# vsislab/Controllable_XGating

Hardware: AMD Instinct MI355X
Metric: decoder timesteps/sec (train fwd+bwd) at batch 128, MSRVTT 26x1536+1024 (higher is better)
Workload: dtype f32; 1 GPU; configs[1]: 1xMI355X batch 128 per GPU teacher-forced XE train, 26 frames x (1536+1024), hidden 512, att 1536, emb 468, vocab 20000, seq_len 20 (T=21), fp32; global_batch=128, per_gpu_batch=128, parallelism=dp1, gemm_precision=fp32, zero_grad=fused into the update, launch=eager kernel launches

## Files before the change

controllable_xgating_amd/csrc/xg_heads.hip:

```cpp
#include "xg_common.h"
#include "xg_kernels.h"
#include "xg_select.h"
#include <type_traits>
#include <cstdlib>

namespace {

constexpr int RT = 1024;

__device__ __forceinline__ float block_max(float v, float* red) {
    v = wave_max(v);
    const int lane = threadIdx.x & 63, wave = threadIdx.x >> 6;
    __syncthreads();
    if (lane == 0) red[wave] = v;
    __syncthreads();
    float r = red[0];
    for (int i = 1; i < (int)(blockDim.x >> 6); ++i) r = fmaxf(r, red[i]);
    return r;
}
__device__ __forceinline__ float block_sum(float v, float* red) {
    v = wave_sum(v);
    const int lane = threadIdx.x & 63, wave = threadIdx.x >> 6;
    __syncthreads();
    if (lane == 0) red[wave] = v;
// ... 147 lines not shown
    s = (mx == -INFINITY) ? 0.f : s * expf(mx - gmx);
    s = block_sum(s, red);
    if (threadIdx.x == 0) {
        const float lse = gmx + logf(s);
        lse_out[i] = lse;
        const float m = mask[(size_t)b * T + t] * (mask2 ? mask2[(size_t)b * T + t] : 1.f);
        const int64_t tg = tgt_of(seq, b, t, T, roll);
        atomicAdd(sums2, -(x[tg] - lse) * m);
        atomicAdd(sums2 + 1, m);
    }
}
__global__ void __launch_bounds__(RT) xent_fwd_kernel(const float* __restrict__ logits, int ld, const int64_t* seq,
                                                        const float* mask, const float* mask2, int B, int T, int V,
                                                        int roll, float* lse_out, float* sums2, int row0) {
    __shared__ float red[RT / 64];
    const int i = row0 + blockIdx.x, t = i / B, b = i % B;
    const float* x = logits + (size_t)i * ld;
    float mx = -INFINITY, s = 0.f;
    for (int v0 = threadIdx.x; v0 < V; v0 += 8 * RT) {
        float xv[8];
#pragma unroll
        for (int j = 0; j < 8; ++j) { const int v = v0 + j * RT; xv[j] = v < V ? x[v] : -INFINITY; }
        float bm = xv[0];
#pragma unroll
        for (int j = 1; j < 8; ++j) bm = fmaxf(bm, xv[j]);
        if (bm > mx) { s *= expf(mx - bm); mx = bm; }
        if (mx > -INFINITY) {
#pragma unroll
            for (int j = 0; j < 8; ++j) s += expf(xv[j] - mx);
        }
    }
    xent_row_finish(mx, s, red, x, i, b, t, T, seq, mask, mask2, roll, lse_out, sums2);
}
template <int NV4>
__global__ void __launch_bounds__(RT) xent_fwd_reg_kernel(const float* __restrict__ logits, int ld, const int64_t* seq,
                                                            const float* mask, const float* mask2, int B, int T, int V,
                                                            int roll, float* lse_out, float* sums2, int row0) {
    __shared__ float red[RT / 64];
    const int i = row0 + blockIdx.x, t = i / B, b = i % B;
    const float* x = logits + (size_t)i * ld;
    float4 xv[NV4];
#pragma unroll
    for (int j = 0; j < NV4; ++j) {
        const int v = (threadIdx.x + j * RT) * 4;
        if (v + 3 < V) xv[j] = *reinterpret_cast<const float4*>(x + v);
        else {
            xv[j].x = v < V ? x[v] : -INFINITY;         xv[j].y = v + 1 < V ? x[v + 1] : -INFINITY;
            xv[j].z = v + 2 < V ? x[v + 2] : -INFINITY; xv[j].w = -INFINITY;
        }
    }
    float mx = -INFINITY;
#pragma unroll
    for (int j = 0; j < NV4; ++j) mx = fmaxf(fmaxf(mx, fmaxf(xv[j].x, xv[j].y)), fmaxf(xv[j].z, xv[j].w));
    float s = 0.f;
    if (mx > -INFINITY) {
#pragma unroll
        for (int j = 0; j < NV4; ++j) s += (expf(xv[j].x - mx) + expf(xv[j].y - mx)) + (expf(xv[j].z - mx) + expf(xv[j].w - mx));
    }
    xent_row_finish(mx, s, red, x, i, b, t, T, seq, mask, mask2, roll, lse_out, sums2);
}
template <bool BF>
__global__ void __launch_bounds__(RT) xent_bwd_kernel(float* __restrict__ logits, int ld, const int64_t* seq,
                                                        const float* mask, const float* mask2, int B, int T, int V,
                                                        int roll, const float* lse, const float* sums2,
                                                        const float* scale_dev, float scale, int row0, unsigned short* d16) {
    const int i = row0 + blockIdx.x, t = i / B, b = i % B;
    float* x = logits + (size_t)i * ld;
    const float m = mask[(size_t)b * T + t] * (mask2 ? mask2[(size_t)b * T + t] : 1.f);
    const float coef = (scale_dev ? scale_dev[0] : 1.f) * scale * m / sums2[1];
    const int64_t tg = tgt_of(seq, b, t, T, roll);
    const float l = lse[i];
    for (int v = threadIdx.x; v < V; v += RT) {
        const float pv = expf(x[v] - l);
        const float gv = coef * (pv - (v == tg ? 1.f : 0.f));
        x[v] = gv;
        if (BF) {
            unsigned u = __float_as_uint(gv);
            u += 0x7FFFu + ((u >> 16) & 1u);
            d16[(size_t)i * ld + v] = (unsigned short)(u >> 16);
        }
    }
}

template <int NV4, bool BF>
__global__ void __launch_bounds__(RT) xent_bwd_reg_kernel(float* __restrict__ logits, int ld, const int64_t* seq,
                                                            const float* mask, const float* mask2, int B, int T, int V,
                                                            int roll, const float* lse, const float* sums2,
                                                            const float* scale_dev, float scale, int row0, unsigned short* d16) {
    const int i = row0 + blockIdx.x, t = i / B, b = i % B;
    float* x = logits + (size_t)i * ld;
    float4 xv[NV4];
#pragma unroll
// ... 1037 lines not shown
    else if (npt <= 16) hipLaunchKernelGGL((log_softmax_reg_kernel<16>), dim3(rows), dim3(RT), 0, st, in, ldin, out, ldout, V, inner, outer, pm);
    else if (npt <= 24) hipLaunchKernelGGL((log_softmax_reg_kernel<24>), dim3(rows), dim3(RT), 0, st, in, ldin, out, ldout, V, inner, outer, pm);
    else hipLaunchKernelGGL(log_softmax_kernel, dim3(rows), dim3(RT), 0, st, in, ldin, out, ldout, V, inner, outer, pm);
    XG_CHECK_LAUNCH();
    return XG_OK;
}
int xgk_log_softmax_bwd(hipStream_t st, const float* dlogp, const float* logp, int ldp, float* dlogits, int ldd,
                        int rows, int V, int inner, int outer, int permute) {
    if (rows <= 0) return XG_OK;
    const int npt = xg_cdiv(V, RT);
    if (npt <= 8) hipLaunchKernelGGL((log_softmax_bwd_reg_kernel<8>), dim3(rows), dim3(RT), 0, st, dlogp, logp, ldp, dlogits, ldd, V, inner, outer, permute);
    else if (npt <= 16) hipLaunchKernelGGL((log_softmax_bwd_reg_kernel<16>), dim3(rows), dim3(RT), 0, st, dlogp, logp, ldp, dlogits, ldd, V, inner, outer, permute);
    else if (npt <= 24) hipLaunchKernelGGL((log_softmax_bwd_reg_kernel<24>), dim3(rows), dim3(RT), 0, st, dlogp, logp, ldp, dlogits, ldd, V, inner, outer, permute);
    else hipLaunchKernelGGL(log_softmax_bwd_kernel, dim3(rows), dim3(RT), 0, st, dlogp, logp, ldp, dlogits, ldd, V, inner, outer, permute);
    XG_CHECK_LAUNCH();
    return XG_OK;
}
int xgk_nll_fwd(hipStream_t st, const float* logp, const int64_t* target, const float* mask, const float* mask2,
                int B, int T, int V, int roll, float* out2) {
    if (hipMemsetAsync(out2, 0, 2 * sizeof(float), st) != hipSuccess) return XG_EHIP;
    hipLaunchKernelGGL(nll_fwd_kernel, dim3(xg_cdiv(B * T, 256)), dim3(256), 0, st, logp, target, mask, mask2, B, T, V,
                       roll, out2);
    XG_CHECK_LAUNCH();
    return XG_OK;
}
int xgk_nll_bwd(hipStream_t st, const int64_t* target, const float* mask, const float* mask2, int B, int T, int V,
                int roll, const float* sums, float scale, const float* scale_dev, float* dlogp) {
    if (hipMemsetAsync(dlogp, 0, sizeof(float) * (size_t)B * T * V, st) != hipSuccess) return XG_EHIP;
    hipLaunchKernelGGL(nll_bwd_kernel, dim3(xg_cdiv(B * T, 256)), dim3(256), 0, st, target, mask, mask2, B, T, V, roll,
                       sums, scale, scale_dev, dlogp);
    XG_CHECK_LAUNCH();
    return XG_OK;
}
int xgk_xent_fwd(hipStream_t st, const float* logits, int ld, const int64_t* seq, const float* mask,
                 const float* mask2, int B, int T, int V, int roll, float* lse, float* sums2, int row0, int nrows,
                 bool zero_sums) {
    if (zero_sums && hipMemsetAsync(sums2, 0, 2 * sizeof(float), st) != hipSuccess) return XG_EHIP;
    if (nrows < 0) nrows = B * T - row0;
    if (nrows <= 0) return XG_OK;
    const bool al = ((uintptr_t)logits % 16 == 0) && ld % 4 == 0;
#define XG_XENT_REG(NV4_) hipLaunchKernelGGL((xent_fwd_reg_kernel<NV4_>), dim3(nrows), dim3(RT), 0, st, logits, ld, seq, mask, mask2, B, T, V, roll, lse, sums2, row0)
    if (al && V <= 2 * 4096) XG_XENT_REG(2);
    else if (al && V <= 5 * 4096) XG_XENT_REG(5);
    else if (al && V <= 8 * 4096) XG_XENT_REG(8);
    else hipLaunchKernelGGL(xent_fwd_kernel, dim3(nrows), dim3(RT), 0, st, logits, ld, seq, mask, mask2, B, T, V, roll, lse, sums2, row0);
#undef XG_XENT_REG
    XG_CHECK_LAUNCH();
    return XG_OK;
}
int xgk_xent_bwd(hipStream_t st, float* logits_inout, int ld, const int64_t* seq, const float* mask,
                 const float* mask2, int B, int T, int V, int roll, const float* lse, const float* sums2,
                 const float* scale_dev, float scale, int row0, int nrows, unsigned short* d16) {
    if (nrows < 0) nrows = B * T - row0;
    if (nrows <= 0) return XG_OK;
    const bool al = ((uintptr_t)logits_inout % 16 == 0) && ld % 4 == 0 && (!d16 || (uintptr_t)d16 % 8 == 0);
#define XG_XENT_BREG(NV4_) do { \
        if (d16) hipLaunchKernelGGL((xent_bwd_reg_kernel<NV4_, true>), dim3(nrows), dim3(RT), 0, st, logits_inout, ld, seq, mask, mask2, B, T, V, \
                                    roll, lse, sums2, scale_dev, scale, row0, d16); \
        else hipLaunchKernelGGL((xent_bwd_reg_kernel<NV4_, false>), dim3(nrows), dim3(RT), 0, st, logits_inout, ld, seq, mask, mask2, B, T, V, \
                                roll, lse, sums2, scale_dev, scale, row0, d16); } while (0)
    if (al && V > 1024 && V <= 2 * 4096) XG_XENT_BREG(2);
    else if (al && V > 1024 && V <= 5 * 4096) XG_XENT_BREG(5);
    else if (al && V > 1024 && V <= 8 * 4096) XG_XENT_BREG(8);
    else if (d16) hipLaunchKernelGGL(xent_bwd_kernel<true>, dim3(nrows), dim3(RT), 0, st, logits_inout, ld, seq, mask, mask2, B, T, V, roll,
                                     lse, sums2, scale_dev, scale, row0, d16);
    else hipLaunchKernelGGL(xent_bwd_kernel<false>, dim3(nrows), dim3(RT), 0, st, logits_inout, ld, seq, mask, mask2, B, T, V, roll,
                            lse, sums2, scale_dev, scale, row0, d16);
#undef XG_XENT_BREG
    XG_CHECK_LAUNCH();
    return XG_OK;
}
int xgk_choose(hipStream_t st, const float* logp, int B, int V, int mode, const float* uniforms,
               const int64_t* forced, int64_t forced_stride, float temperature, int64_t* tok, float* tok_logp) {
    hipLaunchKernelGGL(choose_kernel, dim3(B), dim3(RT), 0, st, logp, V, mode, uniforms, forced, forced_stride,
// ... 124 lines not shown
```

controllable_xgating_amd/csrc/xg_kernels.h:

```cpp
#pragma once
#include "xg_common.h"
#include "xg_select.h"
#include "xg_beam_core.h"
#include "xg_gemm_route.h"
#include <cstddef>
#include <type_traits>

int xgk_gemm(hipStream_t st, int mode, bool transA, bool transB, int M, int N, int K, const float* A, int lda,
             const float* B, int ldb, float* C, int ldc, const float* bias, bool relu, bool accumulate);
int xgk_gemm_cs(hipStream_t st, int mode, bool transA, bool transB, int M, int N, int K, const float* A, int lda,
                const float* B, int ldb, float* C, int ldc, const float* bias, bool relu, bool accumulate, float* cs1, float* cs2,
                float* cs3);
int xgk_gemm_x(hipStream_t st, int mode, bool transA, bool transB, int M, int N, int K, const float* A, const unsigned short* A16,
               int lda, const float* B, const unsigned short* B16, int ldb, float* C, int ldc, const float* bias, bool relu,
               bool accumulate, float* cs1 = nullptr, float* cs2 = nullptr, float* cs3 = nullptr);
struct XgGemmPtrs {
    const float* A; const float* B; float* C; const float* bias;
    const unsigned short* A16; const unsigned short* B16;
    float* cs[3];
};
#ifdef XG_DIAG
int xgk_gemm_run(hipStream_t st, bool wide_forced, int mode, bool transA, bool transB, int M, int N, int K, int lda, int ldb, int ldc,
                 bool relu, bool accumulate, const XgGemmPtrs& p, const XgGemmTuning* tune = nullptr, XgGemmRoute* launched = nullptr);
#else
// ... 196 lines not shown
int xgk_attn_fwd(hipStream_t st, const float* p, const float* vproj, const float* V, const float* w, float* alpha,
                 float* af, int B, int K, int R, int A, bool half_cu = false);
int xgk_attn_fwd_group(hipStream_t st, const float* p, const float* vproj, const float* V, const float* w, float* alpha,
                       float* af, int B, int S, int K, int R, int A);
int xgk_attn_bwd(hipStream_t st, const float* daf, int lddaf, const float* p, const float* vproj, const float* V,
                 const float* w, const float* alpha, float* de, float* dp, int B, int K, int R, int A);
int xgk_attn_bwd_post(hipStream_t st, const float* P , const float* vproj, const float* w,
                      const float* DE , float* dvproj, float* dw, int T, int B, int K, int A);
int xgk_attn_post_dV(hipStream_t st, const float* P, const float* vproj, const float* w, const float* DE, float* dvproj, float* dw,
                     const float* ALPHA, const float* DAF, int lddaf, int64_t daf_tstride, float* dV, int T, int B, int K, int A, int R);
int xgk_attn_dV(hipStream_t st, const float* ALPHA , const float* DAF , int lddaf,
                int64_t daf_tstride, float* dV, int T, int B, int K, int R, bool accumulate);
constexpr int XGK_ATTN_BWD_GROUP = 4;
int xgk_attn_bwd_group(hipStream_t st, const float* daf, int lddaf, const float* p, const float* vproj, const float* V, const float* w,
                       const float* alpha, float* de, float* dp, int B, int Q, int K, int R, int A);
int xgk_attn_bwd_group_form(const float* daf, int lddaf, const float* p, const float* vproj, const float* V, const float* w,
                            const float* dp, int K, int R, int A);
int xgk_attn_post_dV_group(hipStream_t st, const float* P , const float* vproj, const float* w, const float* DE ,
                           float* dvproj, float* dw, const float* ALPHA , const float* DAF, int lddaf, int64_t daf_tstride,
                           float* dV, int T, int B, int Q, int K, int A, int R);
int xgk_rows_sum_group(hipStream_t st, const float* in, float* out, int B, int Q, int R);

int xgk_log_softmax(hipStream_t st, const float* in, int ldin, float* out, int ldout, int rows, int V, int inner,
                    int outer, bool permute);
int xgk_log_softmax_bwd(hipStream_t st, const float* dlogp, const float* logp, int ldp, float* dlogits, int ldd,
                        int rows, int V, int inner, int outer, int permute);
int xgk_nll_fwd(hipStream_t st, const float* logp, const int64_t* target, const float* mask, const float* mask2,
                int B, int T, int V, int roll, float* out2);
int xgk_nll_bwd(hipStream_t st, const int64_t* target, const float* mask, const float* mask2, int B, int T, int V,
                int roll, const float* sums, float scale, const float* scale_dev, float* dlogp);
int xgk_xent_fwd(hipStream_t st, const float* logits, int ld, const int64_t* seq, const float* mask,
                 const float* mask2, int B, int T, int V, int roll, float* lse, float* sums2, int row0 = 0,
                 int nrows = -1, bool zero_sums = true);
int xgk_xent_bwd(hipStream_t st, float* logits_inout, int ld, const int64_t* seq, const float* mask,
                 const float* mask2, int B, int T, int V, int roll, const float* lse, const float* sums2,
                 const float* scale_dev, float scale, int row0 = 0, int nrows = -1, unsigned short* d16 = nullptr);
int xgk_choose(hipStream_t st, const float* logp, int B, int V, int mode, const float* uniforms,
               const int64_t* forced, int64_t forced_stride, float temperature, int64_t* tok, float* tok_logp);
int xgk_rollout_step(hipStream_t st, int B, const RollStepArgs& a);
int xgk_rollout_finalize(hipStream_t st, const int32_t* maxf, int32_t* n_steps, int Tm1, int nparts);
bool xgk_vocab_select_ok(int B, int R, int V, const float* H, int ldh, const float* W);
int xgk_vocab_tile_width(int V);
int xgk_vocab_part(hipStream_t st, int B, int R, int V, const float* H, int ldh, const float* W, const float* bias, float* logits,
                   int wr_rows, float* part, float temperature);
RollSelectArgs xgk_roll_select_args(const RollStepArgs& r, const float* part);
int xgk_roll_select(hipStream_t st, int B, const RollStepArgs& r, const float* part);
int xgk_rollout_trunc(hipStream_t st, int B, const RollStepArgs& r, const RollTruncArgs& q);
int xgk_rollout_dlogits_lse(hipStream_t st, float* logits, const float* lse, const int64_t* tok, const float* dslp,
                            int64_t dstride, int B, int V, int steps);
constexpr int XG_COMPACT_MAX = 48;
struct CompactEntry { float* dst; const float* src; int64_t dst_block, src_pitch, total; };
struct CompactArgs { int n; int start[XG_COMPACT_MAX + 1]; CompactEntry e[XG_COMPACT_MAX]; };
int xgk_compact(hipStream_t st, CompactArgs& a);
int xgk_ss_select(hipStream_t st, const int64_t* seq, int T, int t, int B, const float* u_sel, float ss_prob,
                  const int64_t* sampled, int64_t* tok);
struct SsChoiceArgs {
    const float* logits;
    const float* part;
    const float* u_sel;
    const float* u_tok;
    const int64_t* seq;
    const float* table;
    int64_t* tok;
    int64_t* tok_out;
    float* xt;
    float ss_prob;
// ... 39 lines not shown
```

controllable_xgating_amd/csrc/xg_model.hip:

```cpp
#include "xg_common.h"
#include <cstring>
#include "xg_kernels.h"
#include "../../include/xgate_beam.h"
#include "../../include/xgate_control.h"
#include "../../include/xgate_truncate.h"
#include "../../include/xgate_score.h"
#include "../../include/xgate_beam_control.h"
#include "../../include/xgate_beam_allow.h"
#include "../../include/xgate_beam_rules.h"
#include "../../include/xgate_beam_diverse.h"
#include "../../include/xgate_pair.h"
#include "../../include/xgate_train_video.h"
#include "../../include/xgate_scst_video.h"
#include "../../include/xgate_ss.h"

#include <new>
#include <cstdlib>

namespace {

constexpr int XG_NEV = 64, XG_NRING = 56;
struct XgAux { uint32_t magic; int device; hipStream_t s = nullptr, s2 = nullptr; hipEvent_t ev[XG_NEV]; };
constexpr uint32_t XG_AUX_MAGIC = 0x58474158u;
XgAux* aux_of(const XgRun* run) {
// ... 149 lines not shown
    do { if (hipMemsetAsync((ptr), 0, sizeof(float) * (size_t)(nfloats), (st)) != hipSuccess) return XG_EHIP; } while (0)
#define COPY(st, dst, src, nfloats) \
    do { if (hipMemcpyAsync((dst), (src), sizeof(float) * (size_t)(nfloats), hipMemcpyDeviceToDevice, (st)) != hipSuccess) return XG_EHIP; } while (0)
inline int record_prof(void* event, hipStream_t st) {
    return (!event || hipEventRecord(static_cast<hipEvent_t>(event), st) == hipSuccess) ? XG_OK : XG_EHIP;
}

inline int gemm_nn(hipStream_t st, int mode, int M, int N, int Kc, const float* dY, int lddy, const float* W, int ldw,
                   float* dX, int lddx, bool acc) {
    return xgk_gemm(st, mode, false, false, M, N, Kc, dY, lddy, W, ldw, dX, lddx, nullptr, false, acc);
}
inline int gemm_tn(hipStream_t st, int mode, int Mrows, int N, int K, const float* dY, int lddy, const float* X, int ldx,
                   float* dW, int lddw) {
    return xgk_gemm(st, mode, true, false, N, K, Mrows, dY, lddy, X, ldx, dW, lddw, nullptr, false, true);
}

inline int gemm_tn_cs(hipStream_t st, int mode, int Mrows, int N, int K, const float* dY, int lddy, const float* X, int ldx,
                      float* dW, int lddw, float* b1, float* b2 = nullptr, float* b3 = nullptr) {
    return xgk_gemm_cs(st, mode, true, false, N, K, Mrows, dY, lddy, X, ldx, dW, lddw, nullptr, false, true, b1, b2, b3);
}

inline const unsigned short* m16(const Ws& w, const float* p) {
    return (w.gm == 1 && w.sh16 && p >= w.base_f && p < w.end_f) ? w.sh16 + (p - w.base_f) : nullptr;
}
inline int cvt16(hipStream_t st, const Ws& w, const float* p, size_t n) {
    if (w.gm != 1 || n == 0) return XG_OK;
    if (!w.sh16) return XG_OK;
    const unsigned short* dst = m16(w, p);
    if (!dst) return XG_EINVAL;
    return xgk_cvt_bf16(st, p, const_cast<unsigned short*>(dst), n);
}
inline const unsigned short* w16(const Ws& w, int which) {
    return (w.gm == 1 && w.packed && w.pk.dtype == 1) ? w.pk.w16[which] : nullptr;
}
inline int lin16(hipStream_t st, int mode, int M, int N, int K, const float* X, const unsigned short* X16, int ldx, const float* W,
                 const unsigned short* W16, const float* bias, float* Y, int ldy, bool relu = false, bool acc = false) {
    return xgk_gemm_x(st, mode, false, true, M, N, K, X, X16, ldx, W, W16, K, Y, ldy, bias, relu, acc);
}
inline int nn16(hipStream_t st, int mode, int M, int N, int Kc, const float* dY, const unsigned short* dY16, int lddy, const float* W,
                const unsigned short* W16, int ldw, float* dX, int lddx, bool acc) {
    return xgk_gemm_x(st, mode, false, false, M, N, Kc, dY, dY16, lddy, W, W16, ldw, dX, lddx, nullptr, false, acc);
}
inline int tn16(hipStream_t st, int mode, int Mrows, int N, int K, const float* dY, const unsigned short* dY16, int lddy, const float* X,
                const unsigned short* X16, int ldx, float* dW, int lddw, float* b1 = nullptr, float* b2 = nullptr, float* b3 = nullptr) {
    return xgk_gemm_x(st, mode, true, false, N, K, Mrows, dY, dY16, lddy, X, X16, ldx, dW, lddw, nullptr, false, true, b1, b2, b3);
}

inline SkSeg seg_nt(const float* A, int lda, const float* W, int ldw, int K) {
    SkSeg s{}; s.A = A; s.B = W; s.lda = lda; s.ldb = ldw; s.K = K; s.b_ncontig = 0; return s;
}
inline SkSeg seg_nn(const float* dY, int lddy, const float* W, int ldw, int Kc) {
    SkSeg s{}; s.A = dY; s.B = W; s.lda = lddy; s.ldb = ldw; s.K = Kc; s.b_ncontig = 1; return s;
}
inline SkSeg seg_nt(const Ws& w, int which, const float* A, int lda, const float* W, int ldw, int K) {
    SkSeg s = seg_nt(A, lda, W, ldw, K);
    if (w.packed) { s.Bp = w.pk.m[which]; s.nck = w.pk.nck[which]; }
    return s;
}
inline SkSeg seg_nn(const Ws& w, int which, const float* dY, int lddy, const float* W, int ldw, int Kc) {
    SkSeg s = seg_nn(dY, lddy, W, ldw, Kc);
    if (w.packed) { s.Bp = w.pk.m[which]; s.nck = w.pk.nck[which]; }
    return s;
}
inline void allow_split(SkArgs& sk, int j, const Ws& w) { sk.job[j].ksplit_ok = 1; sk.job[j].tickets = w.tickets + j * SKPART_INTS; }
inline int zero_tickets(hipStream_t st, const Ws& w, int njobs) {
    return hipMemsetAsync(w.tickets, 0, sizeof(int32_t) * njobs * SKPART_INTS, st) == hipSuccess ? XG_OK : XG_EHIP;
// ... 520 lines not shown
    const size_t BR = (size_t)B * R;
    if (!step_scratch_ok(w, false, rows_per_video > 0) || (rows_per_video > 0) != (enc != nullptr)) return XG_EINVAL;
    const Ws& vw = enc ? *enc : w;
    if (!enc) XG_TRY(init_and_vproj(ss, d, p, x.feat_mask, w));
    XG_TRY(zero_dsync(st, w));
    XG_TRY(ss.join());
    const int th = (ss.overlap() && T >= 4) ? T / 2 : 0;
    const bool fwd_bg = th > 0 && w.gm == 0;
    static const char* chunk_env = xg_diag_env("XG_LOGIT_CHUNK");
    int chunk = 3, tail = 2;
    if (chunk_env) sscanf(chunk_env, "%d,%d", &chunk, &tail);
    const bool chunked = fwd_bg && chunk > 0 && tail > 0;
    const int last_cut = chunked ? T - tail : th;
    int done = 0;
    *logit_rows_done = 0;
    XG_TRY(record_prof(run.prof_event0, st));
    for (int t = 0; t < T; ++t) {
        StepIO s = step_io_at(w, d, t);
        s.pre1 = w.PRE1 + (size_t)t * B * 4 * R; s.mask = x.seq_mask + t; s.ldm = T; s.half_attn = fwd_bg;
        s.rows_per_video = rows_per_video;
        XG_TRY(core_step(st, d, p, run, w, vw.Venc, vw.vproj, s));
        const int n = t + 1;
        bool cut;
        if (!chunked) cut = th > 0 && n == th;
        else if (n < last_cut) cut = n % chunk == 0 && last_cut - n >= 2;
        else cut = n == last_cut && n - done >= 2;
        if (cut) {
            const int rows = (n - done) * B, row0 = done * B;
            const float* Hc = w.H2 + BR + (size_t)row0 * R;
            XG_TRY(ss.fork());
            XG_TRY(cvt16(ss.aux, w, Hc, (size_t)rows * R));
            XG_TRY(lin16(ss.aux, w.gm | (fwd_bg ? XGK_GEMM_BG : 0), rows, d.V, R, Hc, m16(w, Hc), R, p.logit_w,
                         w16(w, W16_LOGIT), p.logit_b, w.LOGITS + (size_t)row0 * d.V, d.V));
            if (early_loss)
                XG_TRY(xgk_xent_fwd(ss.aux, w.LOGITS, d.V, x.seq, x.seq_mask, nullptr, B, T, d.V, 1, w.LSE, w.sums, row0, rows, false));
            done = n;
            *logit_rows_done = done * B;
        }
    }
    return record_prof(run.prof_event1, st);
}

int classifier_fwd(hipStream_t st, const XgDims& d, const XgParams& p, const XgRun& run, Ws& w, int rows) {
    const float* Hout = w.H2 + (size_t)d.B * d.R;
    XG_TRY(xgk_linear(st, w.gm, rows, d.H, d.R, Hout, d.R, p.cls0_w, p.cls0_b, w.HC, d.H, true));
    XG_TRY(xgk_gate_fwd(st, w.HC, d.H, nullptr, 0, 0, nullptr, 0, rows, d.H, xg_make_drop(&run, XG_SITE_CLS, 0), d.B, 1 << 30, 1, d.B));
    return xgk_linear(st, w.gm, rows, d.C, d.H, w.HC, d.H, p.cls3_w, p.cls3_b, w.CL, d.C);
}

int heads_fwd_logits(Streams& ss, const XgDims& d, const XgParams& p, const XgRun& run, Ws& w, int rows, int rows_done, bool cls = true) {
    hipStream_t st = ss.main;
    const int R = d.R;
    const float* Hlate = w.H2 + (size_t)d.B * R + (size_t)rows_done * R;
    XG_TRY(cvt16(st, w, Hlate, (size_t)(rows - rows_done) * R));
    XG_TRY(lin16(st, w.gm, rows - rows_done, d.V, R, Hlate, m16(w, Hlate), R, p.logit_w, w16(w, W16_LOGIT), p.logit_b,
                 w.LOGITS + (size_t)rows_done * d.V, d.V));
    if (cls) XG_TRY(classifier_fwd(st, d, p, run, w, rows));
    return ss.join();
}

int decoder_bwd_core(Streams& ss, const XgDims& d, const XgParams& p, const XgParams& g, const XgBatch& x,
                     const XgRun& run, Ws& w, const float* mask, int ldm, int mask_tstride, const int64_t* tok,
                     int tok_bstride, int tok_tstride, int rows_per_video = 0, Ws* enc = nullptr) {
    hipStream_t st = ss.main;
    if ((rows_per_video > 0) != (enc != nullptr) || (rows_per_video > 0 && d.B % rows_per_video != 0)) return XG_EINVAL;
    Ws& vw = enc ? *enc : w;
    const int B = d.B, K = d.K, R = d.R, A = d.A, E = d.E, T = d.T, TB = T * B;
    const int Bv = rows_per_video > 0 ? B / rows_per_video : B, N = Bv * K;
// ... 164 lines not shown
            }
            XG_TRY(gemm_tn_cs(sj, w.gm, Bv, R, R, gst[j], R, vw.vbar, R, gw[j], R, gb[j]));
        }
    }
    XG_TRY(wgrads_chain2(sx, 0, wg_hi));
    XG_TRY(wgrads_chain1(s1, 0, wg_hi));
    XG_TRY(ss.wait_mark2(wg_mark));
    XG_TRY(xgk_gate_bwd(s1, w.DPOSG, R, w.GP, R, x.pos_feats, R, B, w.DGP, R, nullptr, 0, false, TB, R,
                        xg_make_drop(&run, XG_SITE_DGATE, 0)));
    XG_TRY(gemm_tn_cs(s1, w.gm, TB, R, E, w.DGP, R, w.Xe, E, g.dgate_w, E, g.dgate_b));
    XG_TRY(gemm_nn(s1, w.gm, TB, E, R, w.DGP, R, p.dgate_w, E, w.DXe, E, true));
    XG_TRY(xgk_embed_scatter_add(s1, g.embed_w, E, tok, B, tok_bstride, tok_tstride, TB, d.V, w.DXe, E));
    XG_TRY(ss.fork());
    if (w.gm == 1) {
        XG_TRY(tn16(sx, w.gm, N, A, R, vw.DVPROJ, m16(vw, vw.DVPROJ), A, vw.Venc, m16(vw, vw.Venc), R, g.v2a_w, R));
        XG_TRY(xgk_colsum3(sx, vw.DVPROJ, A, N, A, g.v2a_b, nullptr, nullptr));
    } else {
        XG_TRY(tn16(sx, w.gm, N, A, R, vw.DVPROJ, m16(vw, vw.DVPROJ), A, vw.Venc, m16(vw, vw.Venc), R, g.v2a_w, R, g.v2a_b));
    }
    XG_TRY(ss.chain2_into_aux());
    if (ss.grad_event && hipEventRecord(ss.grad_event, sx) != hipSuccess) return XG_EHIP;
    return XG_OK;
}

int zero_backward_block(Streams& ss, Ws& w) {
    w.zeroed = false;
    if (!ss.overlap()) return XG_OK;
    XG_TRY(ss.fork2());
    if (hipMemsetAsync(w.zblock, 0, w.zbytes, ss.aux2) != hipSuccess) return XG_EHIP;
    w.zeroed = true;
    return XG_OK;
}

struct XentBwd { const int64_t* seq; const float* mask; const float* dloss_dev; };
int heads_bwd(Streams& ss, const XgDims& d, const XgParams& p, const XgParams& g, const XgRun& run, Ws& w, int rows,
              bool have_cls, const XentBwd* xent = nullptr) {
    hipStream_t st = ss.main;
    const int B = d.B, R = d.R, TB = d.T * B;
    const float* Hout = w.H2 + (size_t)B * R;
    XG_TRY(zero_backward_block(ss, w));
    if (rows < TB) ZERO(st, w.DH2OUT + (size_t)rows * R, (size_t)(TB - rows) * R);
    const int th = (ss.overlap() && !have_cls && rows == TB && d.T >= 4) ? d.T / 2 : 0;
    const int r0 = th * B;
    ss.dh_split_step = th; ss.dh_mark = -1;
    unsigned short* dl16 = const_cast<unsigned short*>(m16(w, w.LOGITS));
    if (xent) XG_TRY(xgk_xent_bwd(st, w.LOGITS, d.V, xent->seq, xent->mask, nullptr, B, d.T, d.V, 1, w.LSE, w.sums,
                                  xent->dloss_dev, 1.0f, r0, rows - r0, dl16));
    else XG_TRY(cvt16(st, w, w.LOGITS, (size_t)rows * d.V));
    XG_TRY(ss.fork());
    if (xent && r0 > 0) XG_TRY(xgk_xent_bwd(ss.aux, w.LOGITS, d.V, xent->seq, xent->mask, nullptr, B, d.T, d.V, 1, w.LSE,
                                            w.sums, xent->dloss_dev, 1.0f, 0, r0, dl16));
    XG_TRY(cvt16(st, w, Hout, (size_t)rows * R));
    const unsigned short* hout16 = m16(w, Hout);
    XG_TRY(nn16(st, w.gm, rows - r0, R, d.V, w.LOGITS + (size_t)r0 * d.V, m16(w, w.LOGITS + (size_t)r0 * d.V), d.V, p.logit_w,
                w16(w, W16_LOGIT), R, w.DH2OUT + (size_t)r0 * R, R, false));
    const int bgm = w.gm | (ss.overlap() && d.K <= 48 ? XGK_GEMM_BG : 0);
    XG_TRY(ss.fork());
    if (th > 0) {
        XG_TRY(nn16(ss.aux, bgm, r0, R, d.V, w.LOGITS, m16(w, w.LOGITS), d.V, p.logit_w, w16(w, W16_LOGIT), R, w.DH2OUT, R, false));
        ss.dh_mark = ss.mark();
        if (ss.dh_mark == -2) return XG_EHIP;
    }
    XG_TRY(tn16(ss.aux, bgm, rows, d.V, R, w.LOGITS, m16(w, w.LOGITS), d.V, Hout, hout16, R, g.logit_w, R, g.logit_b));
    if (ss.grad_event_head) {
        XG_TRY(ss.fork());
        if (hipEventRecord(ss.grad_event_head, ss.aux) != hipSuccess) return XG_EHIP;
    }
    if (have_cls) {
        XG_TRY(gemm_tn_cs(st, w.gm, rows, d.C, d.H, w.DCL, d.C, w.HC, d.H, g.cls3_w, d.H, g.cls3_b));
        XG_TRY(gemm_nn(st, w.gm, rows, d.H, d.C, w.DCL, d.C, p.cls3_w, d.H, w.DHC, d.H, false));
        XG_TRY(xgk_relu_drop_bwd(st, w.DHC, w.HC, (int64_t)rows * d.H, xg_make_drop(&run, XG_SITE_CLS, 0)));
        XG_TRY(gemm_tn_cs(st, w.gm, rows, d.H, R, w.DHC, d.H, Hout, R, g.cls0_w, R, g.cls0_b));
        XG_TRY(gemm_nn(st, w.gm, rows, R, d.H, w.DHC, d.H, p.cls0_w, R, w.DH2OUT, R, true));
    }
    return XG_OK;
}

__global__ void losses_kernel(const float* s, float wc, float* out) {
    const float lx = s[0] / s[1];
    const float lc = s[3] > 0.f ? s[2] / s[3] : 0.f;
    out[0] = lx + wc * lc; out[1] = lx; out[2] = lc;
}

int check(const XgDims* d, const void* ws, size_t ws_bytes, Ws* w) {
// ... 362 lines not shown
        float* xt = w.Xe + (size_t)t * B * E;
        XG_TRY(xgk_embed_gather(st, p->embed_w, E, tok, B, 1, 0, B, d->V, xt, E));
        StepIO s = step_io_at(w, *d, t);
        s.pos = x->pos_feats; s.gp = w.GP + t * BR; s.mask = x->seq_mask + t; s.ldm = T;
        XG_TRY(core_step(st, *d, *p, *run, w, w.Venc, w.vproj, s));
        float* lg = w.LOGITS + (size_t)t * B * d->V;
        XG_TRY(xgk_linear(st, w.gm, B, d->V, R, s.h2o, R, p->logit_w, p->logit_b, lg, d->V));
        XG_TRY(xgk_log_softmax(st, lg, d->V, lg, d->V, B, d->V, 1, 1, false));
    }
    XG_TRY(xgk_log_softmax(st, w.LOGITS, d->V, logp, d->V, TB, d->V, B, T, true));
    XG_TRY(classifier_fwd(st, *d, *p, *run, w, TB));
    if (cat_logp) XG_TRY(xgk_log_softmax(st, w.CL, d->C, cat_logp, d->C, TB, d->C, B, T, true));
    return XG_OK;
}

extern "C" int xg_backward_ss(void* stream, const XgDims* d, const XgParams* p, const XgParams* g, const XgBatch* x,
                              const XgRun* run, void* ws, size_t ws_bytes, const float* dlogp, const float* dcat_logp) {
    Ws w; XG_TRY(open_ws(d, ws, ws_bytes, run, &w));
    if (!p || !g || !x || !x->seq || !x->seq_mask) return XG_EINVAL;
    hipStream_t st = (hipStream_t)stream;
    XG_TRY(dlogits_from_dlogp(st, *d, w, dlogp, dcat_logp, true));
    Streams ss(st, run);
    return backward_tail(ss, *d, *d, *p, *g, *x, *run, w, dcat_logp != nullptr, nullptr, x->seq_mask, d->T, 1, w.TOK, 1, d->B);
}

extern "C" int xg_xe_loss_fwd(void* stream, const XgDims* d, const XgParams* p, const XgBnState* bn, const XgBatch* x,
                              const int64_t* cap_classes, const float* class_mask, float weight_class, const XgRun* run,
                              void* ws, size_t ws_bytes, float* losses) {
    Ws w; XG_TRY(open_ws(d, ws, ws_bytes, run, &w));
    if (!p || !x || !losses || !x->seq || !x->seq_mask || !x->pos_feats) return XG_EINVAL;
    hipStream_t st = (hipStream_t)stream;
    Streams ss(st, run);
    int rows_done = 0;
    ZERO(st, w.sums, 2);
    static const bool keep_cls = xg_diag_env("XG_KEEP_CLS") != nullptr;
    XG_TRY(forward_xe_front(ss, *d, *p, bn, *x, *run, w, true, &rows_done, cap_classes != nullptr || keep_cls));
    XG_TRY(xgk_xent_fwd(st, w.LOGITS, d->V, x->seq, x->seq_mask, nullptr, d->B, d->T, d->V, 1, w.LSE, w.sums, rows_done, -1, false));
    if (cap_classes) {
        XG_TRY(xgk_xent_fwd(st, w.CL, d->C, cap_classes, x->seq_mask, class_mask, d->B, d->T, d->C, 0, w.LSEC, w.sums + 2));
    } else {
        ZERO(st, w.sums + 2, 2);
    }
    hipLaunchKernelGGL(losses_kernel, dim3(1), dim3(1), 0, st, w.sums, cap_classes ? weight_class : 0.f, losses);
    XG_CHECK_LAUNCH();
    return XG_OK;
}
extern "C" int xg_xe_loss_bwd(void* stream, const XgDims* d, const XgParams* p, const XgParams* g, const XgBatch* x,
                              const int64_t* cap_classes, const float* class_mask, float weight_class,
                              const float* dloss_dev, const XgRun* run, void* ws, size_t ws_bytes) {
    Ws w; XG_TRY(open_ws(d, ws, ws_bytes, run, &w));
    if (!p || !g || !x || !x->seq || !x->seq_mask) return XG_EINVAL;
    hipStream_t st = (hipStream_t)stream;
    const int B = d->B, T = d->T;
    const XentBwd xent{x->seq, x->seq_mask, dloss_dev};
    const bool cls = cap_classes != nullptr && weight_class != 0.f;
    if (cls) {
        COPY(st, w.DCL, w.CL, (size_t)T * B * d->C);
        XG_TRY(xgk_xent_bwd(st, w.DCL, d->C, cap_classes, x->seq_mask, class_mask, B, T, d->C, 0, w.LSEC, w.sums + 2,
                            dloss_dev, weight_class));
    }
    Streams ss(st, run);
    return backward_tail(ss, *d, *d, *p, *g, *x, *run, w, cls, &xent, x->seq_mask, T, 1, x->seq, T, 1);
}

static int videos_once(Streams& es, const XgDims& de, const XgParams& p, const XgBnState* bn, const XgBatch& x, const XgRun& run,
                       Ws& enc, CapBeamRepeatArgs ra, float* const state[4], int rep) {
    XG_TRY(encode_and_init(es, de, p, bn, x, run, enc));
    const float* src[4] = {enc.H1, enc.C1, enc.H2, enc.C2};
    for (int k = 0; k < 4; ++k) ra.e[ra.n++] = CapBeamRepeatEntry{state[k], src[k], (int64_t)de.R};
    return xgk_cap_beam_repeat(es.main, ra, de.B, rep);
}

enum class RolloutForm { Plain, PairVideos, RowsPerVideo };
struct RolloutCall {
    int mode = XG_ROLLOUT_GREEDY;
    const float* uniforms = nullptr; const int64_t* forced = nullptr; float temperature = 1.0f;
    int split = 0;
    float* logits_alt = nullptr; bool used_alt = false;
    RolloutForm form = RolloutForm::Plain;
    const XgDims* d1 = nullptr; Ws* enc = nullptr;
    int rows_per_video = 0;
    bool keep = false;
    bool two_seeds = false; uint32_t seed_greedy = 0;
    const RollTruncArgs* trunc = nullptr;
};
static RolloutCall pair_call(const float* uniforms, float temperature, int n_sample, float* logits_alt = nullptr) {
    RolloutCall c;
// ... 675 lines not shown
    *de = beam_dims(*d, d->B);
    *dm = *d; dm->B = d->B * Q;
    if (run) {
        if (run->gemm_mode != 0) return XG_EINVAL;
        attach_packed(w->enc, *de, run);
        attach_packed(w->row, *dm, run);
    }
    return XG_OK;
}
bool tv_batch_ok(const XgBatch* x) {
    return x && x->feats_rgb && x->feats_opfl && x->feat_mask && x->pos_feats && x->seq && x->seq_mask;
}

}

extern "C" int xgtv_version(void) { return XGTV_VERSION; }

extern "C" size_t xgtv_workspace_bytes(const XgDims* d, int32_t Q) {
    return cc_dims_ok(d, Q) ? tv_carve(*d, Q, nullptr).bytes : 0;
}

extern "C" int xgtv_xe_loss_fwd(void* stream, const XgDims* d, int32_t Q, const XgParams* p, const XgBnState* bn, const XgBatch* x,
                                const int64_t* cap_classes, const float* class_mask, float weight_class, const XgRun* run, void* ws,
                                size_t ws_bytes, float* losses) {
    TrainVideoWs w; XgDims de, dm;
    XG_TRY(tv_open(d, Q, p, run, ws, ws_bytes, &w, &de, &dm));
    if (!run || !tv_batch_ok(x) || !losses) return XG_EINVAL;
    if (!run->train && (!bn || !bn->rgb_mean || !bn->rgb_var || !bn->opfl_mean || !bn->opfl_var)) return XG_EINVAL;
    hipStream_t st = (hipStream_t)stream;
    const int M = dm.B, T = d->T;
    Ws& r = w.row;
    Streams ss(st, run);
    int rows_done = 0;
    ZERO(st, r.sums, 2);
    const bool cls = cap_classes != nullptr;
    XG_TRY(ss.fork());
    XG_TRY(decoder_tokens_xe(ss.aux, dm, *p, *x, *run, r));
    float* const state0[4] = {r.H1, r.C1, r.H2, r.C2};
    XG_TRY(videos_once(ss, de, *p, bn, *x, *run, w.enc, CapBeamRepeatArgs{}, state0, Q));
    XG_TRY(decoder_fwd_xe(ss, dm, *p, *x, *run, r, &rows_done, true, Q, &w.enc));
    XG_TRY(heads_fwd_logits(ss, dm, *p, *run, r, T * M, rows_done, cls));
    XG_TRY(xgk_xent_fwd(st, r.LOGITS, d->V, x->seq, x->seq_mask, nullptr, M, T, d->V, 1, r.LSE, r.sums, rows_done, -1, false));
    if (cap_classes) {
        XG_TRY(xgk_xent_fwd(st, r.CL, d->C, cap_classes, x->seq_mask, class_mask, M, T, d->C, 0, r.LSEC, r.sums + 2));
    } else {
        ZERO(st, r.sums + 2, 2);
    }
    hipLaunchKernelGGL(losses_kernel, dim3(1), dim3(1), 0, st, r.sums, cap_classes ? weight_class : 0.f, losses);
    XG_CHECK_LAUNCH();
    return XG_OK;
}

extern "C" int xgtv_xe_loss_bwd(void* stream, const XgDims* d, int32_t Q, const XgParams* p, const XgParams* g, const XgBatch* x,
                                const int64_t* cap_classes, const float* class_mask, float weight_class, const float* dloss_dev,
                                const XgRun* run, void* ws, size_t ws_bytes) {
    TrainVideoWs w; XgDims de, dm;
    XG_TRY(tv_open(d, Q, p, run, ws, ws_bytes, &w, &de, &dm));
    if (!run || !g || !tv_batch_ok(x) || !dloss_dev) return XG_EINVAL;
    hipStream_t st = (hipStream_t)stream;
    const int M = dm.B, T = d->T;
    Ws& r = w.row;
    const XentBwd xent{x->seq, x->seq_mask, dloss_dev};
    const bool cls = cap_classes != nullptr && weight_class != 0.f;
    if (cls) {
        COPY(st, r.DCL, r.CL, (size_t)T * M * d->C);
        XG_TRY(xgk_xent_bwd(st, r.DCL, d->C, cap_classes, x->seq_mask, class_mask, M, T, d->C, 0, r.LSEC, r.sums + 2, dloss_dev,
                            weight_class));
    }
    Streams ss(st, run);
    XG_TRY(heads_bwd(ss, dm, *p, *g, *run, r, T * M, cls, &xent));
    XG_TRY(decoder_bwd_core(ss, dm, *p, *g, *x, *run, r, x->seq_mask, T, 1, x->seq, T, 1, Q, &w.enc));
    XG_TRY(encoder_bwd(ss, de, *p, *g, *x, *run, w.enc, w.enc.DV));
    return ss.join();
}

extern "C" int xgtv_video_grads(void* stream, const XgDims* d, int32_t Q, const XgParams* p, void* ws, size_t ws_bytes, float* dvproj,
                                float* dV) {
    TrainVideoWs w; XgDims de, dm;
    XG_TRY(tv_open(d, Q, p, nullptr, ws, ws_bytes, &w, &de, &dm));
    if (!dvproj || !dV) return XG_EINVAL;
    const Ws& r = w.row;
    return xgk_attn_post_dV_group((hipStream_t)stream, r.P, w.enc.vproj, p->a2w_w, r.DE, dvproj, nullptr, r.ALPHA, r.DAF, d->R,
                                  (int64_t)dm.B * d->R, dV, d->T, d->B, Q, d->K, d->A, d->R);
}

namespace {

TrainVideoWs sv_carve(const XgDims& d, int S, void* base) {
    TrainVideoWs w{};
    w.enc = carve(beam_dims(d, d.B), base);
    w.enc.sh16 = nullptr; w.enc.bytes = w.enc.core_bytes;
    Carver c{static_cast<char*>(base), w.enc.core_bytes};
    const size_t M = (size_t)d.B * S, K = d.K, R = d.R, A = d.A, E = d.E, V = d.V, T = d.T, TM = T * M;
    Ws& s = w.row;
    carve_step_scratch(c, s, M, R, false);
// ... 155 lines not shown
bool ss_bn_ok(const XgRun* run, const XgBnState* bn) {
    return run->train || (bn && bn->rgb_mean && bn->rgb_var && bn->opfl_mean && bn->opfl_var);
}

}

extern "C" int xgss_version(void) { return XGSS_VERSION; }

extern "C" size_t xgss_workspace_bytes(const XgDims* d, int32_t Q) {
    if (Q < 0 || !ss_dims_ok(d, Q)) return 0;
    return Q == 0 ? carve(*d, nullptr).core_bytes : ssv_carve(*d, Q, nullptr).bytes;
}

extern "C" int xgss_xe_loss_fwd(void* stream, const XgDims* d, int32_t Q, const XgParams* p, const XgBnState* bn, const XgBatch* x,
                                const int64_t* cap_classes, const float* class_mask, float weight_class, float ss_prob,
                                const float* u_sel, const float* u_tok, const XgRun* run, void* ws, size_t ws_bytes, float* losses,
                                int64_t* tok_out) {
    SsWs o;
    XG_TRY(ss_open(d, Q, p, run, ws, ws_bytes, &o));
    if (!tv_batch_ok(x) || !losses || !tok_out || !ss_bn_ok(run, bn)) return XG_EINVAL;
    if (!(ss_prob >= 0.f && ss_prob <= 1.f) || (run->train && ss_prob > 0.f && (!u_sel || !u_tok))) return XG_EINVAL;
    hipStream_t st = (hipStream_t)stream;
    const int M = o.dm.B, T = d->T;
    Ws& r = *o.row;
    Streams ss(st, run);
    if (Q == 0) {
        XG_TRY(encode_and_init(ss, o.de, *p, bn, *x, *run, r));
    } else {
        float* const state0[4] = {r.H1, r.C1, r.H2, r.C2};
        XG_TRY(videos_once(ss, o.de, *p, bn, *x, *run, *o.enc, CapBeamRepeatArgs{}, state0, Q));
    }
    XG_TRY(ss_decoder_loop(ss, o.dm, *p, *x, *run, r, Q, Q > 0 ? o.enc : nullptr, ss_prob, u_sel, u_tok, tok_out));
    XG_TRY(ss.join());
    XG_TRY(xgk_xent_fwd(st, r.LOGITS, d->V, x->seq, x->seq_mask, nullptr, M, T, d->V, 1, r.LSE, r.sums, 0, -1, true));
    if (cap_classes) {
        XG_TRY(classifier_fwd(st, o.dm, *p, *run, r, T * M));
        XG_TRY(xgk_xent_fwd(st, r.CL, d->C, cap_classes, x->seq_mask, class_mask, M, T, d->C, 0, r.LSEC, r.sums + 2));
    } else {
        ZERO(st, r.sums + 2, 2);
    }
    hipLaunchKernelGGL(losses_kernel, dim3(1), dim3(1), 0, st, r.sums, cap_classes ? weight_class : 0.f, losses);
    XG_CHECK_LAUNCH();
    return XG_OK;
}

extern "C" int xgss_xe_loss_bwd(void* stream, const XgDims* d, int32_t Q, const XgParams* p, const XgParams* g, const XgBatch* x,
                                const int64_t* cap_classes, const float* class_mask, float weight_class, const float* dloss_dev,
                                const XgRun* run, void* ws, size_t ws_bytes) {
    SsWs o;
    XG_TRY(ss_open(d, Q, p, run, ws, ws_bytes, &o));
    if (!g || !tv_batch_ok(x) || !dloss_dev) return XG_EINVAL;
    hipStream_t st = (hipStream_t)stream;
    const int M = o.dm.B, T = d->T;
    Ws& r = *o.row;
    const XentBwd xent{x->seq, x->seq_mask, dloss_dev};
    const bool cls = cap_classes != nullptr && weight_class != 0.f;
    if (cls) {
        COPY(st, r.DCL, r.CL, (size_t)T * M * d->C);
        XG_TRY(xgk_xent_bwd(st, r.DCL, d->C, cap_classes, x->seq_mask, class_mask, M, T, d->C, 0, r.LSEC, r.sums + 2, dloss_dev,
                            weight_class));
    }
    Streams ss(st, run);
    if (Q == 0) return backward_tail(ss, *d, *d, *p, *g, *x, *run, r, cls, &xent, x->seq_mask, T, 1, r.TOK, 1, M);
    XG_TRY(heads_bwd(ss, o.dm, *p, *g, *run, r, T * M, cls, &xent));
    XG_TRY(decoder_bwd_core(ss, o.dm, *p, *g, *x, *run, r, x->seq_mask, T, 1, r.TOK, 1, M, Q, o.enc));
    XG_TRY(encoder_bwd(ss, o.de, *p, *g, *x, *run, *o.enc, o.enc->DV));
    return ss.join();
}
```

Baseline: 513,300 decoder timesteps/s.

## Form cross-entropy logit gradients in the forward pass to skip a second logits read

```diff
diff --git a/controllable_xgating_amd/csrc/xg_heads.hip b/controllable_xgating_amd/csrc/xg_heads.hip
--- a/controllable_xgating_amd/csrc/xg_heads.hip
+++ b/controllable_xgating_amd/csrc/xg_heads.hip
@@ -203,13 +203,13 @@
     }
     xent_row_finish(mx, s, red, x, i, b, t, T, seq, mask, mask2, roll, lse_out, sums2);
 }
-template <int NV4>
-__global__ void __launch_bounds__(RT) xent_fwd_reg_kernel(const float* __restrict__ logits, int ld, const int64_t* seq,
+template <int NV4, bool GRAD>
+__global__ void __launch_bounds__(RT) xent_fwd_reg_kernel(float* __restrict__ logits, int ld, const int64_t* seq,
                                                             const float* mask, const float* mask2, int B, int T, int V,
                                                             int roll, float* lse_out, float* sums2, int row0) {
     __shared__ float red[RT / 64];
     const int i = row0 + blockIdx.x, t = i / B, b = i % B;
-    const float* x = logits + (size_t)i * ld;
+    float* x = logits + (size_t)i * ld;
     float4 xv[NV4];
 #pragma unroll
     for (int j = 0; j < NV4; ++j) {
@@ -228,7 +228,54 @@
 #pragma unroll
         for (int j = 0; j < NV4; ++j) s += (expf(xv[j].x - mx) + expf(xv[j].y - mx)) + (expf(xv[j].z - mx) + expf(xv[j].w - mx));
     }
-    xent_row_finish(mx, s, red, x, i, b, t, T, seq, mask, mask2, roll, lse_out, sums2);
+    if (!GRAD) { xent_row_finish(mx, s, red, x, i, b, t, T, seq, mask, mask2, roll, lse_out, sums2); return; }
+    const float gmx = block_max(mx, red);
+    s = (mx == -INFINITY) ? 0.f : s * expf(mx - gmx);
+    s = block_sum(s, red);
+    const float l = gmx + logf(s);
+    const float m = mask[(size_t)b * T + t] * (mask2 ? mask2[(size_t)b * T + t] : 1.f);
+    const float coef = m / sums2[1];
+    const int tg = (int)tgt_of(seq, b, t, T, roll);
+    if (threadIdx.x == 0) lse_out[i] = l;
+#pragma unroll
+    for (int j = 0; j < NV4; ++j) {
+        const int v = (threadIdx.x + j * RT) * 4;
+        if (tg >= v && tg < v + 4 && tg < V) {
+            const float xt = tg == v ? xv[j].x : tg == v + 1 ? xv[j].y : tg == v + 2 ? xv[j].z : xv[j].w;
+            atomicAdd(sums2, -(xt - l) * m);
+        }
+        float4 gq;
+        gq.x = coef * (expf(xv[j].x - l) - (v == tg ? 1.f : 0.f));
+        gq.y = coef * (expf(xv[j].y - l) - (v + 1 == tg ? 1.f : 0.f));
+        gq.z = coef * (expf(xv[j].z - l) - (v + 2 == tg ? 1.f : 0.f));
+        gq.w = coef * (expf(xv[j].w - l) - (v + 3 == tg ? 1.f : 0.f));
+        if (v + 3 < V) *reinterpret_cast<float4*>(x + v) = gq;
+        else {
+            const float ga[3] = {gq.x, gq.y, gq.z};
+            for (int q = 0; q < 3 && v + q < V; ++q) x[v + q] = ga[q];
+        }
+    }
+}
+__global__ void __launch_bounds__(RT) mask_sum_kernel(const float* mask, const float* mask2, int n, float* sums2) {
+    __shared__ float red[RT / 64];
+    float a = 0.f;
+    for (int i = threadIdx.x; i < n; i += RT) a += mask[i] * (mask2 ? mask2[i] : 1.f);
+    a = block_sum(a, red);
+    if (threadIdx.x == 0) { sums2[0] = 0.f; sums2[1] = a; }
+}
+__global__ void __launch_bounds__(RT) xent_scale_kernel(float* __restrict__ dlogits, int ld, int V, const float* scale_dev) {
+    const float sc = scale_dev[0];
+    if (sc == 1.0f) return;
+    float* x = dlogits + (size_t)blockIdx.x * ld;
+    for (int v = threadIdx.x * 4; v < V; v += RT * 4) {
+        if (v + 3 < V) {
+            float4 q = *reinterpret_cast<const float4*>(x + v);
+            q.x *= sc; q.y *= sc; q.z *= sc; q.w *= sc;
+            *reinterpret_cast<float4*>(x + v) = q;
+        } else {
+            for (int e = v; e < V; ++e) x[e] *= sc;
+        }
+    }
 }
 template <bool BF>
 __global__ void __launch_bounds__(RT) xent_bwd_kernel(float* __restrict__ logits, int ld, const int64_t* seq,
@@ -1332,14 +1379,43 @@
     XG_CHECK_LAUNCH();
     return XG_OK;
 }
-int xgk_xent_fwd(hipStream_t st, const float* logits, int ld, const int64_t* seq, const float* mask,
+bool xgk_xent_grad_ok(const float* logits, int ld, int V) {
+    return ((uintptr_t)logits % 16 == 0) && ld % 4 == 0 && V > 1024 && V <= 8 * 4096;
+}
+int xgk_xent_mask_sum(hipStream_t st, const float* mask, const float* mask2, int n, float* sums2) {
+    hipLaunchKernelGGL(mask_sum_kernel, dim3(1), dim3(RT), 0, st, mask, mask2, n, sums2);
+    XG_CHECK_LAUNCH();
+    return XG_OK;
+}
+int xgk_xent_fwd_grad(hipStream_t st, float* logits_inout, int ld, const int64_t* seq, const float* mask,
+                      const float* mask2, int B, int T, int V, int roll, float* lse, float* sums2, int row0, int nrows) {
+    if (!xgk_xent_grad_ok(logits_inout, ld, V)) return XG_EINVAL;
+    if (nrows < 0) nrows = B * T - row0;
+    if (nrows <= 0) return XG_OK;
+#define XG_XENT_GREG(NV4_) hipLaunchKernelGGL((xent_fwd_reg_kernel<NV4_, true>), dim3(nrows), dim3(RT), 0, st, logits_inout, ld, seq, mask, mask2, B, T, V, roll, lse, sums2, row0)
+    if (V <= 2 * 4096) XG_XENT_GREG(2);
+    else if (V <= 5 * 4096) XG_XENT_GREG(5);
+    else XG_XENT_GREG(8);
+#undef XG_XENT_GREG
+    XG_CHECK_LAUNCH();
+    return XG_OK;
+}
+int xgk_xent_scale(hipStream_t st, float* dlogits, int ld, int rows, int V, const float* scale_dev) {
+    if (rows <= 0) return XG_OK;
+    if (!scale_dev || (uintptr_t)dlogits % 16 != 0 || ld % 4 != 0) return XG_EINVAL;
+    hipLaunchKernelGGL(xent_scale_kernel, dim3(rows), dim3(RT), 0, st, dlogits, ld, V, scale_dev);
+    XG_CHECK_LAUNCH();
+    return XG_OK;
+}
+int xgk_xent_fwd(hipStream_t st, const float* logits_in, int ld, const int64_t* seq, const float* mask,
                  const float* mask2, int B, int T, int V, int roll, float* lse, float* sums2, int row0, int nrows,
                  bool zero_sums) {
     if (zero_sums && hipMemsetAsync(sums2, 0, 2 * sizeof(float), st) != hipSuccess) return XG_EHIP;
     if (nrows < 0) nrows = B * T - row0;
     if (nrows <= 0) return XG_OK;
+    float* logits = const_cast<float*>(logits_in);
     const bool al = ((uintptr_t)logits % 16 == 0) && ld % 4 == 0;
-#define XG_XENT_REG(NV4_) hipLaunchKernelGGL((xent_fwd_reg_kernel<NV4_>), dim3(nrows), dim3(RT), 0, st, logits, ld, seq, mask, mask2, B, T, V, roll, lse, sums2, row0)
+#define XG_XENT_REG(NV4_) hipLaunchKernelGGL((xent_fwd_reg_kernel<NV4_, false>), dim3(nrows), dim3(RT), 0, st, logits, ld, seq, mask, mask2, B, T, V, roll, lse, sums2, row0)
     if (al && V <= 2 * 4096) XG_XENT_REG(2);
     else if (al && V <= 5 * 4096) XG_XENT_REG(5);
     else if (al && V <= 8 * 4096) XG_XENT_REG(8);
diff --git a/controllable_xgating_amd/csrc/xg_kernels.h b/controllable_xgating_amd/csrc/xg_kernels.h
--- a/controllable_xgating_amd/csrc/xg_kernels.h
+++ b/controllable_xgating_amd/csrc/xg_kernels.h
@@ -252,6 +252,11 @@
 int xgk_xent_fwd(hipStream_t st, const float* logits, int ld, const int64_t* seq, const float* mask,
                  const float* mask2, int B, int T, int V, int roll, float* lse, float* sums2, int row0 = 0,
                  int nrows = -1, bool zero_sums = true);
+bool xgk_xent_grad_ok(const float* logits, int ld, int V);
+int xgk_xent_mask_sum(hipStream_t st, const float* mask, const float* mask2, int n, float* sums2);
+int xgk_xent_fwd_grad(hipStream_t st, float* logits_inout, int ld, const int64_t* seq, const float* mask,
+                      const float* mask2, int B, int T, int V, int roll, float* lse, float* sums2, int row0 = 0, int nrows = -1);
+int xgk_xent_scale(hipStream_t st, float* dlogits, int ld, int rows, int V, const float* scale_dev);
 int xgk_xent_bwd(hipStream_t st, float* logits_inout, int ld, const int64_t* seq, const float* mask,
                  const float* mask2, int B, int T, int V, int roll, const float* lse, const float* sums2,
                  const float* scale_dev, float scale, int row0 = 0, int nrows = -1, unsigned short* d16 = nullptr);
diff --git a/controllable_xgating_amd/csrc/xg_model.hip b/controllable_xgating_amd/csrc/xg_model.hip
--- a/controllable_xgating_amd/csrc/xg_model.hip
+++ b/controllable_xgating_amd/csrc/xg_model.hip
@@ -205,6 +205,20 @@
 }
 inline const unsigned short* w16(const Ws& w, int which) {
     return (w.gm == 1 && w.packed && w.pk.dtype == 1) ? w.pk.w16[which] : nullptr;
+}
+bool xent_grad_in_fwd(const XgDims& d, const XgRun& run, const Ws& w) {
+    static const bool two_pass = xg_diag_env("XG_XENT_TWO_PASS") != nullptr;
+    return !two_pass && w.gm != 1 && run.save != 0 && xgk_xent_grad_ok(w.LOGITS, d.V, d.V);
+}
+int xent_begin(hipStream_t st, const XgDims& d, const XgBatch& x, const XgRun& run, Ws& w) {
+    if (xent_grad_in_fwd(d, run, w)) return xgk_xent_mask_sum(st, x.seq_mask, nullptr, d.T * d.B, w.sums);
+    ZERO(st, w.sums, 2);
+    return XG_OK;
+}
+int xent_rows(hipStream_t st, const XgDims& d, const XgBatch& x, const XgRun& run, Ws& w, int row0, int nrows) {
+    if (xent_grad_in_fwd(d, run, w))
+        return xgk_xent_fwd_grad(st, w.LOGITS, d.V, x.seq, x.seq_mask, nullptr, d.B, d.T, d.V, 1, w.LSE, w.sums, row0, nrows);
+    return xgk_xent_fwd(st, w.LOGITS, d.V, x.seq, x.seq_mask, nullptr, d.B, d.T, d.V, 1, w.LSE, w.sums, row0, nrows, false);
 }
 inline int lin16(hipStream_t st, int mode, int M, int N, int K, const float* X, const unsigned short* X16, int ldx, const float* W,
                  const unsigned short* W16, const float* bias, float* Y, int ldy, bool relu = false, bool acc = false) {
@@ -791,8 +805,7 @@
             XG_TRY(cvt16(ss.aux, w, Hc, (size_t)rows * R));
             XG_TRY(lin16(ss.aux, w.gm | (fwd_bg ? XGK_GEMM_BG : 0), rows, d.V, R, Hc, m16(w, Hc), R, p.logit_w,
                          w16(w, W16_LOGIT), p.logit_b, w.LOGITS + (size_t)row0 * d.V, d.V));
-            if (early_loss)
-                XG_TRY(xgk_xent_fwd(ss.aux, w.LOGITS, d.V, x.seq, x.seq_mask, nullptr, B, T, d.V, 1, w.LSE, w.sums, row0, rows, false));
+            if (early_loss) XG_TRY(xent_rows(ss.aux, d, x, run, w, row0, rows));
             done = n;
             *logit_rows_done = done * B;
         }
@@ -1023,7 +1036,7 @@
     return XG_OK;
 }
 
-struct XentBwd { const int64_t* seq; const float* mask; const float* dloss_dev; };
+struct XentBwd { const int64_t* seq; const float* mask; const float* dloss_dev; bool formed; };
 int heads_bwd(Streams& ss, const XgDims& d, const XgParams& p, const XgParams& g, const XgRun& run, Ws& w, int rows,
               bool have_cls, const XentBwd* xent = nullptr) {
     hipStream_t st = ss.main;
@@ -1035,12 +1048,14 @@
     const int r0 = th * B;
     ss.dh_split_step = th; ss.dh_mark = -1;
     unsigned short* dl16 = const_cast<unsigned short*>(m16(w, w.LOGITS));
-    if (xent) XG_TRY(xgk_xent_bwd(st, w.LOGITS, d.V, xent->seq, xent->mask, nullptr, B, d.T, d.V, 1, w.LSE, w.sums,
-                                  xent->dloss_dev, 1.0f, r0, rows - r0, dl16));
-    else XG_TRY(cvt16(st, w, w.LOGITS, (size_t)rows * d.V));
+    const bool two_pass = xent && !xent->formed;
+    if (two_pass) XG_TRY(xgk_xent_bwd(st, w.LOGITS, d.V, xent->seq, xent->mask, nullptr, B, d.T, d.V, 1, w.LSE, w.sums,
+                                      xent->dloss_dev, 1.0f, r0, rows - r0, dl16));
+    else if (!xent) XG_TRY(cvt16(st, w, w.LOGITS, (size_t)rows * d.V));
+    else if (xent->dloss_dev) XG_TRY(xgk_xent_scale(st, w.LOGITS, d.V, rows, d.V, xent->dloss_dev));
     XG_TRY(ss.fork());
-    if (xent && r0 > 0) XG_TRY(xgk_xent_bwd(ss.aux, w.LOGITS, d.V, xent->seq, xent->mask, nullptr, B, d.T, d.V, 1, w.LSE,
-                                            w.sums, xent->dloss_dev, 1.0f, 0, r0, dl16));
+    if (two_pass && r0 > 0) XG_TRY(xgk_xent_bwd(ss.aux, w.LOGITS, d.V, xent->seq, xent->mask, nullptr, B, d.T, d.V, 1, w.LSE,
+                                                w.sums, xent->dloss_dev, 1.0f, 0, r0, dl16));
     XG_TRY(cvt16(st, w, Hout, (size_t)rows * R));
     const unsigned short* hout16 = m16(w, Hout);
     XG_TRY(nn16(st, w.gm, rows - r0, R, d.V, w.LOGITS + (size_t)r0 * d.V, m16(w, w.LOGITS + (size_t)r0 * d.V), d.V, p.logit_w,
@@ -1469,10 +1484,10 @@
     hipStream_t st = (hipStream_t)stream;
     Streams ss(st, run);
     int rows_done = 0;
-    ZERO(st, w.sums, 2);
+    XG_TRY(xent_begin(st, *d, *x, *run, w));
     static const bool keep_cls = xg_diag_env("XG_KEEP_CLS") != nullptr;
     XG_TRY(forward_xe_front(ss, *d, *p, bn, *x, *run, w, true, &rows_done, cap_classes != nullptr || keep_cls));
-    XG_TRY(xgk_xent_fwd(st, w.LOGITS, d->V, x->seq, x->seq_mask, nullptr, d->B, d->T, d->V, 1, w.LSE, w.sums, rows_done, -1, false));
+    XG_TRY(xent_rows(st, *d, *x, *run, w, rows_done, -1));
     if (cap_classes) {
         XG_TRY(xgk_xent_fwd(st, w.CL, d->C, cap_classes, x->seq_mask, class_mask, d->B, d->T, d->C, 0, w.LSEC, w.sums + 2));
     } else {
@@ -1489,7 +1504,7 @@
     if (!p || !g || !x || !x->seq || !x->seq_mask) return XG_EINVAL;
     hipStream_t st = (hipStream_t)stream;
     const int B = d->B, T = d->T;
-    const XentBwd xent{x->seq, x->seq_mask, dloss_dev};
+    const XentBwd xent{x->seq, x->seq_mask, dloss_dev, xent_grad_in_fwd(*d, *run, w)};
     const bool cls = cap_classes != nullptr && weight_class != 0.f;
     if (cls) {
         COPY(st, w.DCL, w.CL, (size_t)T * B * d->C);
@@ -2231,7 +2246,7 @@
     Ws& r = w.row;
     Streams ss(st, run);
     int rows_done = 0;
-    ZERO(st, r.sums, 2);
+    XG_TRY(xent_begin(st, dm, *x, *run, r));
     const bool cls = cap_classes != nullptr;
     XG_TRY(ss.fork());
     XG_TRY(decoder_tokens_xe(ss.aux, dm, *p, *x, *run, r));
@@ -2239,7 +2254,7 @@
     XG_TRY(videos_once(ss, de, *p, bn, *x, *run, w.enc, CapBeamRepeatArgs{}, state0, Q));
     XG_TRY(decoder_fwd_xe(ss, dm, *p, *x, *run, r, &rows_done, true, Q, &w.enc));
     XG_TRY(heads_fwd_logits(ss, dm, *p, *run, r, T * M, rows_done, cls));
-    XG_TRY(xgk_xent_fwd(st, r.LOGITS, d->V, x->seq, x->seq_mask, nullptr, M, T, d->V, 1, r.LSE, r.sums, rows_done, -1, false));
+    XG_TRY(xent_rows(st, dm, *x, *run, r, rows_done, -1));
     if (cap_classes) {
         XG_TRY(xgk_xent_fwd(st, r.CL, d->C, cap_classes, x->seq_mask, class_mask, M, T, d->C, 0, r.LSEC, r.sums + 2));
     } else {
@@ -2259,7 +2274,7 @@
     hipStream_t st = (hipStream_t)stream;
     const int M = dm.B, T = d->T;
     Ws& r = w.row;
-    const XentBwd xent{x->seq, x->seq_mask, dloss_dev};
+    const XentBwd xent{x->seq, x->seq_mask, dloss_dev, xent_grad_in_fwd(dm, *run, r)};
     const bool cls = cap_classes != nullptr && weight_class != 0.f;
     if (cls) {
         COPY(st, r.DCL, r.CL, (size_t)T * M * d->C);
@@ -2481,7 +2496,8 @@
     }
     XG_TRY(ss_decoder_loop(ss, o.dm, *p, *x, *run, r, Q, Q > 0 ? o.enc : nullptr, ss_prob, u_sel, u_tok, tok_out));
     XG_TRY(ss.join());
-    XG_TRY(xgk_xent_fwd(st, r.LOGITS, d->V, x->seq, x->seq_mask, nullptr, M, T, d->V, 1, r.LSE, r.sums, 0, -1, true));
+    XG_TRY(xent_begin(st, o.dm, *x, *run, r));
+    XG_TRY(xent_rows(st, o.dm, *x, *run, r, 0, -1));
     if (cap_classes) {
         XG_TRY(classifier_fwd(st, o.dm, *p, *run, r, T * M));
         XG_TRY(xgk_xent_fwd(st, r.CL, d->C, cap_classes, x->seq_mask, class_mask, M, T, d->C, 0, r.LSEC, r.sums + 2));
@@ -2502,7 +2518,7 @@
     hipStream_t st = (hipStream_t)stream;
     const int M = o.dm.B, T = d->T;
     Ws& r = *o.row;
-    const XentBwd xent{x->seq, x->seq_mask, dloss_dev};
+    const XentBwd xent{x->seq, x->seq_mask, dloss_dev, xent_grad_in_fwd(o.dm, *run, r)};
     const bool cls = cap_classes != nullptr && weight_class != 0.f;
     if (cls) {
         COPY(st, r.DCL, r.CL, (size_t)T * M * d->C);
```

Result: no change. 516,000 decoder timesteps/s (median of 6 runs) (+0.5%).
